# ajzhai/PEANUT

Hardware: AMD Instinct MI355X
Metric: maps/sec for 480x480x(4+N_cat) prediction fwd, batch 32 (higher is better)
Workload: dtype f32

## Files before the change

peanut_amd/csrc/conv_pw_ares.hip:

```cpp
#include <stdlib.h>

#include "common.h"
#include "conv_common.h"

namespace peanut {

namespace {

typedef const __attribute__((address_space(1))) void* gptr_t;
typedef __attribute__((address_space(3))) void* lptr_t;

__device__ __forceinline__ float load_uncounted(const float* ptr) {
  float v;
  asm volatile("global_load_dword %0, %1, off" : "=v"(v) : "v"(ptr) : "memory");
  return v;
}
template <int CH>
__device__ __forceinline__ void wait_uncounted(const float (&r)[CH], float a, float b) {
  static_assert(CH == 4 || CH == 8, "chunk of 4 or 8 values");
  __builtin_amdgcn_sched_barrier(0);
  if constexpr (CH == 4)
    asm volatile("s_waitcnt vmcnt(0)" ::"v"(r[0]), "v"(r[1]), "v"(r[2]), "v"(r[3]), "v"(a), "v"(b) : "memory");
  else
    asm volatile("s_waitcnt vmcnt(0)" ::"v"(r[0]), "v"(r[1]), "v"(r[2]), "v"(r[3]), "v"(r[4]), "v"(r[5]), "v"(r[6]), "v"(r[7]), "v"(a), "v"(b)
                 : "memory");
  __builtin_amdgcn_sched_barrier(0);
}

template <int NK, bool FLUSH>
__global__ __launch_bounds__(512) void conv_pw_ares_kernel(const ConvKParams p) {
  constexpr int BK = 32, K = NK * BK, TILE = 128 * BK;
  constexpr int CH = 32 / NK;
  static_assert(NK == 4 || NK == 8, "K = 128 or 256");
  __shared__ __attribute__((aligned(1024))) float smem[(NK + 2) * TILE];
  float* const bst = smem + NK * TILE;

  const int tid = threadIdx.x, lane = tid & 63;
  const int wave = __builtin_amdgcn_readfirstlane(tid >> 6);
  const int lr = lane >> 3, lp = lane & 7;
  const int wm = wave >> 2, wn = wave & 3;
  const int li = lane & 31, hi = lane >> 5;
  const bool late = p.phase_shift && wave >= 4;

  const int G = gridDim.x, bid = blockIdx.x;
  const int lw = (bid & 7) * (G >> 3) + (bid >> 3);
  const int NT = p.ntiles;
  const long long U = (long long)p.mtiles * NT;
  const int u0 = (int)(U * lw / G), u1 = (int)(U * (lw + 1) / G);
  if (u0 >= u1) return;

  const int pbn = p.ares_pbn;
  unsigned a_off[2], b_off[2];
#pragma unroll
  for (int j = 0; j < 2; ++j) {
    const int r = (wave * 2 + j) * 8 + lr;
    const int c = lp ^ ((r >> 1) & 7);
    a_off[j] = r * K + c * 4;
    b_off[j] = (r / pbn) * (NK * pbn * BK) + (r % pbn) * BK + c * 4;
  }
  auto dma_a = [&](int mt, int s) {
    const float* base = p.x + (size_t)mt * (128 * K) + s * BK;
#pragma unroll
    for (int j = 0; j < 2; ++j)
      __builtin_amdgcn_global_load_lds((gptr_t)(base + a_off[j]), (lptr_t)(smem + s * TILE + (wave * 2 + j) * 256), 16, 0, 0);
  };
  auto dma_b = [&](int mt, int nt, int kt, int stage) {
    const float* base = p.w + (p.mt_per_group ? (size_t)(mt / p.mt_per_group) * p.w_group_stride : 0) + (size_t)nt * (128 * K) + kt * (pbn * BK);
#pragma unroll
    for (int j = 0; j < 2; ++j)
      __builtin_amdgcn_global_load_lds((gptr_t)(base + b_off[j]), (lptr_t)(bst + stage * TILE + (wave * 2 + j) * 256), 16, 0, 0);
  };

  const int swz = (li >> 1) & 7;
  int sw[4];
#pragma unroll
  for (int ks = 0; ks < 4; ++ks) sw[ks] = ((ks * 2 + hi) ^ swz) * 4;
  const int a_row = (wm * 64 + li) * BK;
  const int b_row = (wn * 32 + li) * BK;

  f32x16 acc[2], acc2[2], prev[2];
#pragma unroll
  for (int t = 0; t < 2; ++t)
#pragma unroll
    for (int r = 0; r < 16; ++r) { acc[t][r] = 0.f; acc2[t][r] = 0.f; prev[t][r] = 0.f; }

  const size_t lane_el = (size_t)(wm * 64 + 4 * hi) * p.cout + wn * 32 + li;
  const bool has_res = p.res != nullptr;
  const size_t rstride = has_res ? (size_t)p.cout : 0;
  const size_t ostride = (size_t)p.cout;
  const float* res_run = has_res ? p.res + lane_el : p.zeros;
  float* out_run = p.y + lane_el;
  const float* prev_sc = p.scale + wn * 32 + li;
  const float* prev_sh = p.shift + wn * 32 + li;
  bool prev_valid = false;
  float scv = 1.f, shv = 0.f;
  const float alpha = p.alpha;
  const bool relu = p.relu != 0;

#define ARES_CHUNK_LOADS(kt)                                                              \
  float resv[CH];                                                                         \
  if ((kt) == 0) {                                                                        \
    scv = load_uncounted(prev_sc);                                                        \
    shv = load_uncounted(prev_sh);                                                        \
  }                                                                                       \
  _Pragma("unroll") for (int i = 0; i < CH; ++i)                                          \
    resv[i] = load_uncounted(res_run + (size_t)(8 * (i >> 2) + (i & 3)) * rstride);       \
  res_run += (size_t)(2 * CH) * rstride;
#define ARES_CHUNK_FINISH(kt)                                                             \
  if (prev_valid) {                                                   \
    _Pragma("unroll") for (int i = 0; i < CH; ++i) {                                      \
      const int idx = (kt) * CH + i;                                                      \
      float v = prev[idx >> 4][idx & 15] * (scv * alpha) + shv;                           \
      v += resv[i];                                                                       \
      if (relu) v = relu_keep_nan(v);                                                     \
      out_run[(size_t)(8 * (i >> 2) + (i & 3)) * ostride] = v;                            \
    }                                                                                     \
  }                                                                                       \
  out_run += (size_t)(2 * CH) * ostride;

  {
    const int mt = u0 / NT, nt = u0 - mt * NT;
#pragma unroll
    for (int s = 0; s < NK; ++s) dma_a(mt, s);
    dma_b(mt, nt, 0, 0);
    asm volatile("s_waitcnt vmcnt(0)" ::: "memory");
    __builtin_amdgcn_s_barrier();
    asm volatile("" ::: "memory");
  }

  int stage = 0;
  for (int u = u0; u < u1; ++u) {
    const int mt = u / NT, nt = u - mt * NT;
    const bool nxt = u + 1 < u1;
    const int mt_n = nxt ? (u + 1) / NT : mt;
    const int nt_n = nxt ? (u + 1) - mt_n * NT : 0;
    const bool refill_next = nxt && mt_n != mt;

    static_for<NK>([&](auto kc) {
      constexpr int kt = decltype(kc)::value;
      const float* const cur_b = bst + stage * TILE;
      const float* const cur_a = smem + kt * TILE;
      const bool more = (kt + 1 < NK) || nxt;
      ARES_CHUNK_LOADS(kt)
      auto request = [&]() {
        if (more) {
          if (kt + 1 < NK) dma_b(mt, nt, kt + 1, stage ^ 1);
          else dma_b(mt_n, nt_n, 0, stage ^ 1);
        }
      };
      if (!late) request();
      __builtin_amdgcn_sched_barrier(0);
      f32x4 af[4][2], bf[4];
#pragma unroll
      for (int j = 0; j < 4; ++j) {
        af[j][0] = *reinterpret_cast<const f32x4*>(cur_a + a_row + sw[j]);
        af[j][1] = *reinterpret_cast<const f32x4*>(cur_a + a_row + 32 * BK + sw[j]);
        bf[j] = *reinterpret_cast<const f32x4*>(cur_b + b_row + sw[j]);
      }
#pragma unroll
      for (int j = 0; j < 2; ++j)
#pragma unroll
        for (int kk = 0; kk < 4; ++kk)
#pragma unroll
          for (int t = 0; t < 2; ++t) acc[t] = __builtin_amdgcn_mfma_f32_32x32x2f32(af[j][t][kk], bf[j][kk], acc[t], 0, 0, 0);
      __builtin_amdgcn_sched_barrier(0);
      if (late) request();
      __builtin_amdgcn_sched_barrier(0);
#pragma unroll
      for (int j = 2; j < 4; ++j)
#pragma unroll
        for (int kk = 0; kk < 4; ++kk)
#pragma unroll
          for (int t = 0; t < 2; ++t) acc[t] = __builtin_amdgcn_mfma_f32_32x32x2f32(af[j][t][kk], bf[j][kk], acc[t], 0, 0, 0);
      if (FLUSH && (kt & 1)) {
#pragma unroll
        for (int t = 0; t < 2; ++t) {
          acc2[t] += acc[t];
#pragma unroll
          for (int r = 0; r < 16; ++r) acc[t][r] = 0.f;
        }
      }
      wait_uncounted<CH>(resv, scv, shv);
      ARES_CHUNK_FINISH(kt)
      if (kt >= 1) { if (refill_next) dma_a(mt_n, kt - 1); }
      asm volatile("s_waitcnt lgkmcnt(0)" ::: "memory");
      __builtin_amdgcn_s_barrier();
      asm volatile("" ::: "memory");
      stage ^= 1;
    });

#pragma unroll
    for (int t = 0; t < 2; ++t) {
      prev[t] = FLUSH ? acc2[t] : acc[t];
#pragma unroll
      for (int r = 0; r < 16; ++r) { acc[t][r] = 0.f; acc2[t][r] = 0.f; }
    }
    {
      const size_t unit_el = (size_t)mt * 128 * p.cout + (size_t)nt * 128 + lane_el;
      res_run = has_res ? p.res + unit_el : p.zeros;
      out_run = p.y + unit_el;
      const int ss_off = (p.mt_per_group && p.ss_group_stride) ? (mt / p.mt_per_group) * p.ss_group_stride : 0;
      prev_sc = p.scale + ss_off + nt * 128 + wn * 32 + li;
      prev_sh = p.shift + ss_off + nt * 128 + wn * 32 + li;
      prev_valid = true;
    }
    if (refill_next) dma_a(mt_n, NK - 1);
  }

  static_for<NK>([&](auto kc) {
    constexpr int kt = decltype(kc)::value;
    ARES_CHUNK_LOADS(kt)
    wait_uncounted<CH>(resv, scv, shv);
    ARES_CHUNK_FINISH(kt)
  });
#undef ARES_CHUNK_LOADS
#undef ARES_CHUNK_FINISH
}

template <int NK, bool FLUSH>
int launch_ares_t(ConvKParams p, hipStream_t stream) {
  int dev = 0, cus = 0;
  if (hipGetDevice(&dev) != hipSuccess || hipDeviceGetAttribute(&cus, hipDeviceAttributeMultiprocessorCount, dev) != hipSuccess || cus < 8)
    return fail(-3, "conv_pw_ares: no current device");
  const long long U = (long long)p.mtiles * p.ntiles;
  long long G = U < cus ? U : cus;
  G -= G % 8;
  if (G < 8) return fail(-2, "conv_pw_ares: launch too small");
  hipLaunchKernelGGL((conv_pw_ares_kernel<NK, FLUSH>), dim3((unsigned)G), dim3(512), 0, stream, p);
  hipError_t e = hipGetLastError();
  if (e != hipSuccess) return fail(-3, std::string("conv_pw_ares launch: ") + hipGetErrorString(e));
  return 0;
}

}

bool conv_pw_uses_ares(int cin, int cout, long long M, int stride, bool two_source, int flush_ktiles, int bn_tile) {
  const bool on = opt(OPT_PW_ARES) != 0;
  const long long min_units = opt(OPT_PW_ARES_MINUNITS);
  if (!on || two_source || (cin != 128 && cin != 256) || stride != 1 || M % 128 != 0 || cout % 128 != 0) return false;
  if (bn_tile != 64 && bn_tile != 128) return false;
  if (flush_ktiles != 0 && flush_ktiles != 2) return false;
  return (M / 128) * (cout / 128) >= min_units;
}

int launch_conv_pw_ares(const ConvKParams& p0, int bn_tile, hipStream_t stream) {
  ConvKParams p = p0;
  p.phase_shift = opt(OPT_PW256_PHASE) != 0;
  p.ares_pbn = bn_tile;
  p.mtiles = p.M / 128;
  p.ntiles = p.cout / 128;
  note_kernel("conv_pw_ares_128x128");
  const bool flush = p.flush == 2;
  if (p.c1 == 256) return flush ? launch_ares_t<8, true>(p, stream) : launch_ares_t<8, false>(p, stream);
  return flush ? launch_ares_t<4, true>(p, stream) : launch_ares_t<4, false>(p, stream);
}

}
```

Measured before the change: 887.8.

## Defer epilogue stores by one chunk via buffer stores to overlap with MFMA

The fused residual epilogue now keeps each chunk's results in registers and issues their stores one chunk later, alongside the next B-tile DMA, instead of storing right after the wait. The stores use raw buffer stores through a resource descriptor; the first tile's descriptor has zero range, which replaces the prev_valid branch. The residual wait leaves one chunk of stores in flight so it no longer blocks on them. An optional trace path timestamps each phase with s_memtime when a compile-time macro is set. The cost is extra registers for the pending values and more complex vmcnt ordering, which could break if the count is wrong.

```diff
diff --git a/peanut_amd/csrc/conv_pw_ares.hip b/peanut_amd/csrc/conv_pw_ares.hip
--- a/peanut_amd/csrc/conv_pw_ares.hip
+++ b/peanut_amd/csrc/conv_pw_ares.hip
@@ -15,17 +15,30 @@
   asm volatile("global_load_dword %0, %1, off" : "=v"(v) : "v"(ptr) : "memory");
   return v;
 }
-template <int CH>
+template <int CH, int LEFT>
 __device__ __forceinline__ void wait_uncounted(const float (&r)[CH], float a, float b) {
   static_assert(CH == 4 || CH == 8, "chunk of 4 or 8 values");
+  static_assert(LEFT == 0 || LEFT == CH, "nothing, or one chunk of stores, left in flight");
   __builtin_amdgcn_sched_barrier(0);
   if constexpr (CH == 4)
-    asm volatile("s_waitcnt vmcnt(0)" ::"v"(r[0]), "v"(r[1]), "v"(r[2]), "v"(r[3]), "v"(a), "v"(b) : "memory");
+    asm volatile("s_waitcnt vmcnt(%6)" ::"v"(r[0]), "v"(r[1]), "v"(r[2]), "v"(r[3]), "v"(a), "v"(b), "n"(LEFT) : "memory");
   else
-    asm volatile("s_waitcnt vmcnt(0)" ::"v"(r[0]), "v"(r[1]), "v"(r[2]), "v"(r[3]), "v"(r[4]), "v"(r[5]), "v"(r[6]), "v"(r[7]), "v"(a), "v"(b)
+    asm volatile("s_waitcnt vmcnt(%10)" ::"v"(r[0]), "v"(r[1]), "v"(r[2]), "v"(r[3]), "v"(r[4]), "v"(r[5]), "v"(r[6]), "v"(r[7]), "v"(a), "v"(b),
+                 "n"(LEFT)
                  : "memory");
   __builtin_amdgcn_sched_barrier(0);
 }
+
+__device__ __forceinline__ __amdgpu_buffer_rsrc_t tile_rsrc(float* base, bool valid) {
+  return __builtin_amdgcn_make_buffer_rsrc(base, (short)0, valid ? 0x7fffffff : 0, 0x00020000);
+}
+
+#ifdef PEANUT_ARES_TRACE
+#define ARES_STAMP(t)                                                              \
+  __builtin_amdgcn_sched_barrier(0);                                               \
+  asm volatile("s_memtime %0\n\ts_waitcnt lgkmcnt(0)" : "=s"(t)::"memory");         \
+  __builtin_amdgcn_sched_barrier(0);
+#endif
 
 template <int NK, bool FLUSH>
 __global__ __launch_bounds__(512) void conv_pw_ares_kernel(const ConvKParams p) {
@@ -85,15 +98,17 @@
     for (int r = 0; r < 16; ++r) { acc[t][r] = 0.f; acc2[t][r] = 0.f; prev[t][r] = 0.f; }
 
   const size_t lane_el = (size_t)(wm * 64 + 4 * hi) * p.cout + wn * 32 + li;
+  const unsigned lane_ob = (unsigned)lane_el * 4u;
   const bool has_res = p.res != nullptr;
   const size_t rstride = has_res ? (size_t)p.cout : 0;
-  const size_t ostride = (size_t)p.cout;
+  const int orow_b = p.cout * 4;
   const float* res_run = has_res ? p.res + lane_el : p.zeros;
-  float* out_run = p.y + lane_el;
   const float* prev_sc = p.scale + wn * 32 + li;
   const float* prev_sh = p.shift + wn * 32 + li;
-  bool prev_valid = false;
-  float scv = 1.f, shv = 0.f;
+  __amdgpu_buffer_rsrc_t st_cur = tile_rsrc(p.y, false), st_old = st_cur;
+  float scv = 1.f, shv = 0.f, pend[CH];
+#pragma unroll
+  for (int i = 0; i < CH; ++i) pend[i] = 0.f;
   const float alpha = p.alpha;
   const bool relu = p.relu != 0;
 
@@ -107,16 +122,17 @@
     resv[i] = load_uncounted(res_run + (size_t)(8 * (i >> 2) + (i & 3)) * rstride);       \
   res_run += (size_t)(2 * CH) * rstride;
 #define ARES_CHUNK_FINISH(kt)                                                             \
-  if (prev_valid) {                                                   \
-    _Pragma("unroll") for (int i = 0; i < CH; ++i) {                                      \
-      const int idx = (kt) * CH + i;                                                      \
-      float v = prev[idx >> 4][idx & 15] * (scv * alpha) + shv;                           \
-      v += resv[i];                                                                       \
-      if (relu) v = relu_keep_nan(v);                                                     \
-      out_run[(size_t)(8 * (i >> 2) + (i & 3)) * ostride] = v;                            \
-    }                                                                                     \
-  }                                                                                       \
-  out_run += (size_t)(2 * CH) * ostride;
+  _Pragma("unroll") for (int i = 0; i < CH; ++i) {                                        \
+    const int idx = (kt) * CH + i;                                                        \
+    float v = prev[idx >> 4][idx & 15] * (scv * alpha) + shv;                             \
+    v += resv[i];                                                                         \
+    if (relu) v = relu_keep_nan(v);                                                       \
+    pend[i] = v;                                                                          \
+  }
+#define ARES_CHUNK_STORES(rsrc, chunk)                                                    \
+  _Pragma("unroll") for (int i = 0; i < CH; ++i)                                          \
+    __builtin_amdgcn_raw_buffer_store_b32(__builtin_bit_cast(unsigned, pend[i]), (rsrc), lane_ob, \
+                                          (2 * CH * (chunk) + 8 * (i >> 2) + (i & 3)) * orow_b, 0);
 
   {
     const int mt = u0 / NT, nt = u0 - mt * NT;
@@ -128,6 +144,11 @@
     asm volatile("" ::: "memory");
   }
 
+#ifdef PEANUT_ARES_TRACE
+  long long tr_sum[5] = {0, 0, 0, 0, 0}, tr_n = 0;
+  unsigned long long t0, t1, t2, t3, t4;
+  ARES_STAMP(t0)
+#endif
   int stage = 0;
   for (int u = u0; u < u1; ++u) {
     const int mt = u / NT, nt = u - mt * NT;
@@ -142,14 +163,19 @@
       const float* const cur_a = smem + kt * TILE;
       const bool more = (kt + 1 < NK) || nxt;
       ARES_CHUNK_LOADS(kt)
-      auto request = [&]() {
+      auto issue = [&]() {
         if (more) {
           if (kt + 1 < NK) dma_b(mt, nt, kt + 1, stage ^ 1);
           else dma_b(mt_n, nt_n, 0, stage ^ 1);
         }
+        if constexpr (kt == 0) { ARES_CHUNK_STORES(st_old, NK - 1) }
+        else { ARES_CHUNK_STORES(st_cur, kt - 1) }
       };
-      if (!late) request();
+      if (!late) issue();
       __builtin_amdgcn_sched_barrier(0);
+#ifdef PEANUT_ARES_TRACE
+      ARES_STAMP(t1)
+#endif
       f32x4 af[4][2], bf[4];
 #pragma unroll
       for (int j = 0; j < 4; ++j) {
@@ -164,7 +190,7 @@
 #pragma unroll
           for (int t = 0; t < 2; ++t) acc[t] = __builtin_amdgcn_mfma_f32_32x32x2f32(af[j][t][kk], bf[j][kk], acc[t], 0, 0, 0);
       __builtin_amdgcn_sched_barrier(0);
-      if (late) request();
+      if (late) issue();
       __builtin_amdgcn_sched_barrier(0);
 #pragma unroll
       for (int j = 2; j < 4; ++j)
@@ -180,12 +206,30 @@
           for (int r = 0; r < 16; ++r) acc[t][r] = 0.f;
         }
       }
-      wait_uncounted<CH>(resv, scv, shv);
+#ifdef PEANUT_ARES_TRACE
+      ARES_STAMP(t2)
+#endif
+      wait_uncounted<CH, CH>(resv, scv, shv);
+#ifdef PEANUT_ARES_TRACE
+      ARES_STAMP(t3)
+#endif
       ARES_CHUNK_FINISH(kt)
       if (kt >= 1) { if (refill_next) dma_a(mt_n, kt - 1); }
+#ifdef PEANUT_ARES_TRACE
+      ARES_STAMP(t4)
+#endif
       asm volatile("s_waitcnt lgkmcnt(0)" ::: "memory");
       __builtin_amdgcn_s_barrier();
       asm volatile("" ::: "memory");
+#ifdef PEANUT_ARES_TRACE
+      {
+        unsigned long long t5;
+        ARES_STAMP(t5)
+        tr_sum[0] += (long long)(t1 - t0); tr_sum[1] += (long long)(t2 - t1); tr_sum[2] += (long long)(t3 - t2);
+        tr_sum[3] += (long long)(t4 - t3); tr_sum[4] += (long long)(t5 - t4); ++tr_n;
+        t0 = t5;
+      }
+#endif
       stage ^= 1;
     });
 
@@ -198,23 +242,34 @@
     {
       const size_t unit_el = (size_t)mt * 128 * p.cout + (size_t)nt * 128 + lane_el;
       res_run = has_res ? p.res + unit_el : p.zeros;
-      out_run = p.y + unit_el;
+      st_old = st_cur;
+      st_cur = tile_rsrc(p.y + (size_t)mt * 128 * p.cout + (size_t)nt * 128, true);
       const int ss_off = (p.mt_per_group && p.ss_group_stride) ? (mt / p.mt_per_group) * p.ss_group_stride : 0;
       prev_sc = p.scale + ss_off + nt * 128 + wn * 32 + li;
       prev_sh = p.shift + ss_off + nt * 128 + wn * 32 + li;
-      prev_valid = true;
     }
     if (refill_next) dma_a(mt_n, NK - 1);
   }
 
+  ARES_CHUNK_STORES(st_old, NK - 1)
   static_for<NK>([&](auto kc) {
     constexpr int kt = decltype(kc)::value;
     ARES_CHUNK_LOADS(kt)
-    wait_uncounted<CH>(resv, scv, shv);
+    wait_uncounted<CH, 0>(resv, scv, shv);
     ARES_CHUNK_FINISH(kt)
+    ARES_CHUNK_STORES(st_cur, kt)
   });
+#ifdef PEANUT_ARES_TRACE
+  if (bid < 16 && lane == 0) {
+    long long* const tr = reinterpret_cast<long long*>(p.partial) + (bid * 8 + wave) * 8;
+    for (int j = 0; j < 5; ++j) tr[j] = tr_sum[j];
+    tr[5] = tr_n;
+    tr[6] = late;
+  }
+#endif
 #undef ARES_CHUNK_LOADS
 #undef ARES_CHUNK_FINISH
+#undef ARES_CHUNK_STORES
 }
 
 template <int NK, bool FLUSH>
```

Result: no change. 890.8 (median of 6 runs) (+0.3%).

## Software-pipeline LDS fragment reads against MFMA issue in ares pointwise conv

Applied to the files above, without the earlier changes.

Replaces the up-front read of all four LDS fragment groups with an interleaved schedule. The next group is read while MFMAs run on the current one, with explicit lgkmcnt waits and sched barriers between steps. The aim is to hide LDS latency behind matrix work and lower register pressure from holding all fragments at once. It also adds optional s_memtime tracing, compiled in only when a trace macro is defined. The extra waits and barriers may constrain the compiler's scheduling.

```diff
diff --git a/peanut_amd/csrc/conv_pw_ares.hip b/peanut_amd/csrc/conv_pw_ares.hip
--- a/peanut_amd/csrc/conv_pw_ares.hip
+++ b/peanut_amd/csrc/conv_pw_ares.hip
@@ -26,6 +26,18 @@
                  : "memory");
   __builtin_amdgcn_sched_barrier(0);
 }
+
+#ifdef PEANUT_ARES_TRACE
+__device__ unsigned long long ares_trace[256 * 8 * 8];
+#define ARES_STAMP(t)                                                                           \
+  __builtin_amdgcn_sched_barrier(0);                                                            \
+  asm volatile("s_memtime %0\n\ts_waitcnt lgkmcnt(0)" : "=s"(t)::"memory");                     \
+  __builtin_amdgcn_sched_barrier(0);
+#define ARES_TRACE(...) __VA_ARGS__
+#else
+#define ARES_STAMP(t)
+#define ARES_TRACE(...)
+#endif
 
 template <int NK, bool FLUSH>
 __global__ __launch_bounds__(512) void conv_pw_ares_kernel(const ConvKParams p) {
@@ -129,6 +141,8 @@
   }
 
   int stage = 0;
+  ARES_TRACE(unsigned long long tr_first = 0; unsigned long long tr_last = 0; unsigned long long tr_sum[4] = {0, 0, 0, 0}; int tr_n = 0;
+             ARES_STAMP(tr_first))
   for (int u = u0; u < u1; ++u) {
     const int mt = u / NT, nt = u - mt * NT;
     const bool nxt = u + 1 < u1;
@@ -141,6 +155,7 @@
       const float* const cur_b = bst + stage * TILE;
       const float* const cur_a = smem + kt * TILE;
       const bool more = (kt + 1 < NK) || nxt;
+      ARES_TRACE(unsigned long long t0, t1, t2, t3, t4; ARES_STAMP(t0))
       ARES_CHUNK_LOADS(kt)
       auto request = [&]() {
         if (more) {
@@ -151,27 +166,37 @@
       if (!late) request();
       __builtin_amdgcn_sched_barrier(0);
       f32x4 af[4][2], bf[4];
-#pragma unroll
-      for (int j = 0; j < 4; ++j) {
+      auto read = [&](int j) {
         af[j][0] = *reinterpret_cast<const f32x4*>(cur_a + a_row + sw[j]);
         af[j][1] = *reinterpret_cast<const f32x4*>(cur_a + a_row + 32 * BK + sw[j]);
         bf[j] = *reinterpret_cast<const f32x4*>(cur_b + b_row + sw[j]);
-      }
-#pragma unroll
-      for (int j = 0; j < 2; ++j)
+        __builtin_amdgcn_sched_barrier(0);
+      };
+      auto mfma = [&](int j) {
 #pragma unroll
         for (int kk = 0; kk < 4; ++kk)
 #pragma unroll
           for (int t = 0; t < 2; ++t) acc[t] = __builtin_amdgcn_mfma_f32_32x32x2f32(af[j][t][kk], bf[j][kk], acc[t], 0, 0, 0);
+      };
+      auto lds_wait = [&]() {
+        __builtin_amdgcn_sched_barrier(0);
+        __builtin_amdgcn_s_waitcnt(0xC07F);
+        __builtin_amdgcn_sched_barrier(0);
+      };
+      read(0);
+      lds_wait();
+      read(1);
+      mfma(0);
+      lds_wait();
+      read(2);
+      mfma(1);
       __builtin_amdgcn_sched_barrier(0);
       if (late) request();
-      __builtin_amdgcn_sched_barrier(0);
-#pragma unroll
-      for (int j = 2; j < 4; ++j)
-#pragma unroll
-        for (int kk = 0; kk < 4; ++kk)
-#pragma unroll
-          for (int t = 0; t < 2; ++t) acc[t] = __builtin_amdgcn_mfma_f32_32x32x2f32(af[j][t][kk], bf[j][kk], acc[t], 0, 0, 0);
+      lds_wait();
+      read(3);
+      mfma(2);
+      lds_wait();
+      mfma(3);
       if (FLUSH && (kt & 1)) {
 #pragma unroll
         for (int t = 0; t < 2; ++t) {
@@ -180,12 +205,17 @@
           for (int r = 0; r < 16; ++r) acc[t][r] = 0.f;
         }
       }
+      ARES_STAMP(t1)
       wait_uncounted<CH>(resv, scv, shv);
+      ARES_STAMP(t2)
       ARES_CHUNK_FINISH(kt)
       if (kt >= 1) { if (refill_next) dma_a(mt_n, kt - 1); }
       asm volatile("s_waitcnt lgkmcnt(0)" ::: "memory");
+      ARES_STAMP(t3)
       __builtin_amdgcn_s_barrier();
       asm volatile("" ::: "memory");
+      ARES_STAMP(t4)
+      ARES_TRACE(tr_sum[0] += t1 - t0; tr_sum[1] += t2 - t1; tr_sum[2] += t3 - t2; tr_sum[3] += t4 - t3; tr_last = t4; ++tr_n;)
       stage ^= 1;
     });
 
@@ -207,6 +237,11 @@
     if (refill_next) dma_a(mt_n, NK - 1);
   }
 
+  ARES_TRACE(if (lane == 0) {
+    unsigned long long* const o = ares_trace + (size_t)(bid * 8 + wave) * 8;
+    o[0] = tr_n; o[1] = tr_last - tr_first;
+    for (int i = 0; i < 4; ++i) o[2 + i] = tr_sum[i];
+  })
   static_for<NK>([&](auto kc) {
     constexpr int kt = decltype(kc)::value;
     ARES_CHUNK_LOADS(kt)
```

After: 890.0 before, 896.3 after, median of 6. Within noise of the previous version (+0.7%).
